# mikwieczorek/centroids-reid

Measured on AMD Instinct MI355X. Metric: train_images_per_sec, higher is better.
Workload: dtype bf16; 1 GPU; ResNet50 256x128 CTL training step: fwd+bwd, centroid-triplet + center + xent, Adam + center SGD (BASELINE configs[1]); P=16, K=4, global_batch=64, num_classes=751, parallelism=single

## Files before the change

centroids-reid_amd/csrc/elementwise.hip:

```cpp
#include "conv_common.hpp"

template <typename T> struct Vec16;
template <> struct Vec16<float> {
  static constexpr int N = 4;
  static __device__ __forceinline__ void load(const float* p, float (&v)[4]) {
    const float4 t = *reinterpret_cast<const float4*>(p); v[0] = t.x; v[1] = t.y; v[2] = t.z; v[3] = t.w;
  }
  static __device__ __forceinline__ void store(float* p, const float (&v)[4]) {
    *reinterpret_cast<float4*>(p) = make_float4(v[0], v[1], v[2], v[3]);
  }
  static __device__ __forceinline__ float rnd(float v) { return v; }
};
template <> struct Vec16<unsigned short> {
  static constexpr int N = 8;
  static __device__ __forceinline__ void load(const unsigned short* p, float (&v)[8]) {
    const uint4 t = *reinterpret_cast<const uint4*>(p);
    const unsigned w[4] = {t.x, t.y, t.z, t.w};
#pragma unroll
    for (int i = 0; i < 4; ++i) { v[2 * i] = __uint_as_float(w[i] << 16); v[2 * i + 1] = __uint_as_float(w[i] & 0xffff0000u); }
  }
  static __device__ __forceinline__ void store(unsigned short* p, const float (&v)[8]) {
    unsigned w[4];
#pragma unroll
    for (int i = 0; i < 4; ++i) w[i] = f32x2_to_bf16x2_bits(v[2 * i], v[2 * i + 1]);
    *reinterpret_cast<uint4*>(p) = make_uint4(w[0], w[1], w[2], w[3]);
  }
  static __device__ __forceinline__ float rnd(float v) { return bf16_bits_to_f32(f32_to_bf16_bits(v)); }
};

template <> struct Vec16<_Float16> {
  static constexpr int N = 8;
  static __device__ __forceinline__ void load(const _Float16* p, float (&v)[8]) {
    const uint4 t = *reinterpret_cast<const uint4*>(p);
    const unsigned w[4] = {t.x, t.y, t.z, t.w};
#pragma unroll
    for (int i = 0; i < 4; ++i) { v[2 * i] = F16T::lo(w[i]); v[2 * i + 1] = F16T::hi(w[i]); }
  }
  static __device__ __forceinline__ void store(_Float16* p, const float (&v)[8]) {
    unsigned w[4];
#pragma unroll
    for (int i = 0; i < 4; ++i) w[i] = F16T::pack2(v[2 * i], v[2 * i + 1]);
    *reinterpret_cast<uint4*>(p) = make_uint4(w[0], w[1], w[2], w[3]);
  }
  static __device__ __forceinline__ float rnd(float v) { return (float)(_Float16)v; }
};

template <int CW>
__global__ __launch_bounds__(1024) void bn2d_finalize_kernel(const float* __restrict__ partial, int rows, int C,
                                                            double count, float* __restrict__ rmean,
                                                            float* __restrict__ rvar, int training, float momentum,
                                                            float eps, const float* __restrict__ gamma,
                                                            const float* __restrict__ beta,
                                                            float* __restrict__ mean_out,
                                                            float* __restrict__ invstd_out,
                                                            float* __restrict__ scale_shift) {
  constexpr int RG = 1024 / CW;
  __shared__ double red[16][2][CW];
  const int cl = threadIdx.x % CW, rg = threadIdx.x / CW;
  const int c = blockIdx.x * CW + cl;
  if (!training) {
    if (rg == 0 && c < C) {
      const float mu = rmean[c], is = 1.0f / sqrtf(rvar[c] + eps);
      mean_out[c] = mu; invstd_out[c] = is;
      const float sc = is * (gamma ? gamma[c] : 1.f);
      scale_shift[c] = sc; scale_shift[C + c] = (beta ? beta[c] : 0.f) - mu * sc;
    }
    return;
  }
  double s1 = 0.0, s2 = 0.0;
  if (c < C)
  {
    int r = rg;
    for (; r + 3 * RG < rows; r += 4 * RG) {
      const float a0 = partial[((int64_t)r * 2) * C + c], b0 = partial[((int64_t)r * 2 + 1) * C + c];
      const float a1 = partial[((int64_t)(r + RG) * 2) * C + c], b1 = partial[((int64_t)(r + RG) * 2 + 1) * C + c];
      const float a2 = partial[((int64_t)(r + 2 * RG) * 2) * C + c], b2 = partial[((int64_t)(r + 2 * RG) * 2 + 1) * C + c];
      const float a3 = partial[((int64_t)(r + 3 * RG) * 2) * C + c], b3 = partial[((int64_t)(r + 3 * RG) * 2 + 1) * C + c];
      s1 += ((double)a0 + (double)a1) + ((double)a2 + (double)a3);
      s2 += ((double)b0 + (double)b1) + ((double)b2 + (double)b3);
    }
    for (; r < rows; r += RG) {
      s1 += (double)partial[((int64_t)r * 2) * C + c];
      s2 += (double)partial[((int64_t)r * 2 + 1) * C + c];
    }
  }
#pragma unroll
  for (int o = CW; o < 64; o <<= 1) { s1 += __shfl_xor(s1, o, 64); s2 += __shfl_xor(s2, o, 64); }
  if ((threadIdx.x & 63) < CW) { red[threadIdx.x >> 6][0][cl] = s1; red[threadIdx.x >> 6][1][cl] = s2; }
  float p_gamma = 1.f, p_beta = 0.f, p_rm = 0.f, p_rv = 0.f;
  if (rg == 0 && c < C) {
    if (gamma) p_gamma = gamma[c];
    if (beta) p_beta = beta[c];
    if (rmean) p_rm = rmean[c];
    if (rvar) p_rv = rvar[c];
  }
  __syncthreads();
  if (rg == 0 && c < C) {
    s1 = 0.0; s2 = 0.0;
#pragma unroll
    for (int q = 0; q < 16; ++q) { s1 += red[q][0][cl]; s2 += red[q][1][cl]; }
    const double mean = s1 / count;
    double var = s2 / count - mean * mean;
    if (var < 0.0) var = 0.0;
    const float mu = (float)mean, is = (float)(1.0 / sqrt(var + (double)eps));
    mean_out[c] = mu;
    invstd_out[c] = is;
    const float sc = is * p_gamma;
    scale_shift[c] = sc; scale_shift[C + c] = p_beta - mu * sc;
    if (rmean) rmean[c] = (1.f - momentum) * p_rm + momentum * (float)mean;
    if (rvar) rvar[c] = (1.f - momentum) * p_rv + momentum * (float)(count > 1.0 ? var * count / (count - 1.0) : var);
  }
}

template <typename T>
__global__ __launch_bounds__(256) void col_stats_kernel(const T* __restrict__ x, int64_t M, int C, int rows_per_block,
                                                        float* __restrict__ partial) {
  constexpr int V = Vec16<T>::N;
  __shared__ float red[2][256 * V];
  const int cpr = C / V, cw = cpr < 32 ? cpr : 32, nrl = 256 / cw;
  const int cch = threadIdx.x % cw, rl = threadIdx.x / cw;
  const int c0 = (blockIdx.x * cw + cch) * V;
  const int64_t r0 = (int64_t)blockIdx.y * rows_per_block, r1 = min(M, r0 + rows_per_block);
  float s1[V], s2[V];
#pragma unroll
  for (int k = 0; k < V; ++k) { s1[k] = 0.f; s2[k] = 0.f; }
  if (c0 < C)
    for (int64_t r = r0 + rl; r < r1; r += nrl) {
// ... 473 lines not shown
__device__ __forceinline__ void store_taps(uint8_t* p, const uint8_t (&bi)[V]) {
  static_assert(V == 4 || V == 8, "16-byte vectors of 4- or 2-byte elements");
  uint32_t lo = (uint32_t)bi[0] | ((uint32_t)bi[1] << 8) | ((uint32_t)bi[2] << 16) | ((uint32_t)bi[3] << 24);
  if constexpr (V == 4) {
    *reinterpret_cast<uint32_t*>(p) = lo;
  } else {
    uint32_t hi = (uint32_t)bi[4] | ((uint32_t)bi[5] << 8) | ((uint32_t)bi[6] << 16) | ((uint32_t)bi[7] << 24);
    *reinterpret_cast<uint2*>(p) = make_uint2(lo, hi);
  }
}
template <typename T>
__global__ __launch_bounds__(256) void maxpool_fwd_kernel(const T* __restrict__ x, int B, int H, int W, int C,
                                                          T* __restrict__ y, uint8_t* __restrict__ idx) {
  constexpr int V = Vec16<T>::N;
  const int OH = H / 2, OW = W / 2, cpr = C / V;
  const int64_t total = (int64_t)B * OH * OW * cpr;
  for (int64_t i = (int64_t)blockIdx.x * 256 + threadIdx.x; i < total; i += (int64_t)gridDim.x * 256) {
    int cc, ox, oy, b;
    if (total < (int64_t)1 << 31) {
      const unsigned u = (unsigned)i, q1 = u / (unsigned)cpr, q2 = q1 / (unsigned)OW;
      cc = (int)(u - q1 * cpr); ox = (int)(q1 - q2 * OW); b = (int)(q2 / (unsigned)OH); oy = (int)(q2 - (unsigned)b * OH);
    } else {
      cc = (int)(i % cpr);
      int64_t p = i / cpr;
      ox = (int)(p % OW); p /= OW;
      oy = (int)(p % OH);
      b = (int)(p / OH);
    }
    float best[V];
    uint8_t bi[V];
#pragma unroll
    for (int k = 0; k < V; ++k) { best[k] = -INFINITY; bi[k] = 0; }
#pragma unroll
    for (int r = 0; r < 3; ++r)
#pragma unroll
      for (int s = 0; s < 3; ++s) {
        const int iy = oy * 2 + r - 1, ix = ox * 2 + s - 1;
        if ((unsigned)iy < (unsigned)H && (unsigned)ix < (unsigned)W) {
          float v[V];
          Vec16<T>::load(x + (((int64_t)b * H + iy) * W + ix) * C + cc * V, v);
#pragma unroll
          for (int k = 0; k < V; ++k)
            if (v[k] > best[k]) { best[k] = v[k]; bi[k] = (uint8_t)(r * 3 + s); }
        }
      }
    Vec16<T>::store(y + i * V, best);
    if (idx) store_taps<V>(idx + i * V, bi);
  }
}

template <typename T>
__global__ __launch_bounds__(256) void bn_apply_maxpool_kernel(const T* __restrict__ x, const float* __restrict__ scale_shift,
                                                               int relu, int B, int H, int W, int C, T* __restrict__ y,
                                                               uint8_t* __restrict__ idx) {
  constexpr int V = Vec16<T>::N;
  const int OH = H / 2, OW = W / 2, cpr = C / V;
  const int64_t total = (int64_t)B * OH * OW * cpr;
  for (int64_t i = (int64_t)blockIdx.x * 256 + threadIdx.x; i < total; i += (int64_t)gridDim.x * 256) {
    int cc, ox, oy, b;
    if (total < (int64_t)1 << 31) {
      const unsigned u = (unsigned)i, q1 = u / (unsigned)cpr, q2 = q1 / (unsigned)OW;
      cc = (int)(u - q1 * cpr); ox = (int)(q1 - q2 * OW); b = (int)(q2 / (unsigned)OH); oy = (int)(q2 - (unsigned)b * OH);
    } else {
      cc = (int)(i % cpr);
      int64_t p = i / cpr;
      ox = (int)(p % OW); p /= OW;
      oy = (int)(p % OH);
      b = (int)(p / OH);
    }
    float sc[V], sh[V], best[V];
    uint8_t bi[V];
#pragma unroll
    for (int k = 0; k < V; ++k) { sc[k] = scale_shift[cc * V + k]; sh[k] = scale_shift[C + cc * V + k]; best[k] = -INFINITY; bi[k] = 0; }
#pragma unroll
    for (int r = 0; r < 3; ++r)
#pragma unroll
      for (int s = 0; s < 3; ++s) {
        const int iy = oy * 2 + r - 1, ix = ox * 2 + s - 1;
        if ((unsigned)iy < (unsigned)H && (unsigned)ix < (unsigned)W) {
          float v[V];
          Vec16<T>::load(x + (((int64_t)b * H + iy) * W + ix) * C + cc * V, v);
#pragma unroll
          for (int k = 0; k < V; ++k) {
            float yv = fmaf(v[k], sc[k], sh[k]);
            if (relu) yv = fmaxf(yv, 0.f);
            yv = Vec16<T>::rnd(yv);
            if (yv > best[k]) { best[k] = yv; bi[k] = (uint8_t)(r * 3 + s); }
          }
        }
      }
    Vec16<T>::store(y + i * V, best);
    if (idx) store_taps<V>(idx + i * V, bi);
  }
}

template <typename T>
__global__ __launch_bounds__(256) void maxpool_bwd_kernel(const T* __restrict__ dy, const uint8_t* __restrict__ idx,
                                                          int B, int H, int W, int C, T* __restrict__ dx) {
  constexpr int V = Vec16<T>::N;
  const int OH = H / 2, OW = W / 2, cpr = C / V;
  const int row = blockIdx.x;
  const int b = row / H, iy = row - b * H;
  T* drow = dx + (int64_t)row * W * C;
  const int nr = (iy & 1) ? 2 : 1;
  const int rr0 = (iy & 1) ? 0 : 1, rstep = 2;
  for (int par = 0; par < 2; ++par) {
    const int ns = par ? 2 : 1, ss0 = par ? 0 : 1;
    for (int v = threadIdx.x; v < (W / 2) * cpr; v += 256) {
      const int ix = 2 * (v / cpr) + par, cc = v % cpr;
      float acc[V];
#pragma unroll
      for (int k = 0; k < V; ++k) acc[k] = 0.f;
      for (int ri = 0; ri < nr; ++ri) {
        const int r = rr0 + ri * rstep, oy = (iy + 1 - r) >> 1;
        if (oy >= OH) continue;
        for (int si = 0; si < ns; ++si) {
          const int sx = ss0 + si * 2, ox = (ix + 1 - sx) >> 1;
          if (ox >= OW) continue;
          const int64_t o = ((((int64_t)b * OH + oy) * OW + ox) * cpr + cc) * V;
          float g[V];
          Vec16<T>::load(dy + o, g);
          uint8_t tap[V];
          if constexpr (V == 8) *reinterpret_cast<uint2*>(tap) = *reinterpret_cast<const uint2*>(idx + o);
          else *reinterpret_cast<unsigned*>(tap) = *reinterpret_cast<const unsigned*>(idx + o);
          const uint8_t want = (uint8_t)(r * 3 + sx);
#pragma unroll
          for (int k = 0; k < V; ++k) acc[k] += (tap[k] == want) ? g[k] : 0.f;
        }
      }
      Vec16<T>::store(drow + ((int64_t)ix * cpr + cc) * V, acc);
    }
  }
}

template <typename T>
__global__ __launch_bounds__(256) void gap_fwd_kernel(const T* __restrict__ x, int HW, int C, float* __restrict__ out,
                                                      int64_t* __restrict__ counter) {
  constexpr int V = Vec16<T>::N;
  __shared__ float red[8][32][V + 1];
  if (counter && blockIdx.x == 0 && blockIdx.y == 0 && threadIdx.x == 0) *counter += 1;
  const int cl = threadIdx.x & 31, rl = threadIdx.x >> 5;
  const int b = blockIdx.y, cc = blockIdx.x * 32 + cl;
  const bool live = cc * V < C;
  float acc[V];
#pragma unroll
  for (int k = 0; k < V; ++k) acc[k] = 0.f;
  if (live) {
    const T* p = x + (int64_t)b * HW * C + cc * V;
    for (int i = rl; i < HW; i += 8) {
      float v[V];
      Vec16<T>::load(p + (int64_t)i * C, v);
#pragma unroll
      for (int k = 0; k < V; ++k) acc[k] += v[k];
    }
  }
#pragma unroll
  for (int k = 0; k < V; ++k) red[rl][cl][k] = acc[k];
  __syncthreads();
  for (int e = threadIdx.x; e < 32 * V; e += 256) {
    const int c2 = e / V, k = e - c2 * V;
    const int ch = (blockIdx.x * 32 + c2) * V + k;
    if (ch < C) {
      float a = 0.f;
#pragma unroll
      for (int q = 0; q < 8; ++q) a += red[q][c2][k];
      out[(int64_t)b * C + ch] = a / (float)HW;
    }
  }
}

template <typename T>
__global__ __launch_bounds__(256) void gap_bwd_kernel(const float* __restrict__ dfeat, int HW, int C, int64_t total_chunks,
                                                      T* __restrict__ dx) {
  constexpr int V = Vec16<T>::N;
  const int cpr = C / V;
  const float inv = 1.0f / (float)HW;
  for (int64_t i = (int64_t)blockIdx.x * 256 + threadIdx.x; i < total_chunks; i += (int64_t)gridDim.x * 256) {
    int cc;
    int64_t b;
    if (total_chunks < (int64_t)1 << 31) { const unsigned u = (unsigned)i; cc = (int)(u % (unsigned)cpr); b = u / (unsigned)(cpr * HW); }
    else { cc = (int)(i % cpr); b = i / ((int64_t)cpr * HW); }
    float v[V];
#pragma unroll
    for (int k = 0; k < V; ++k) v[k] = dfeat[b * C + cc * V + k] * inv;
    Vec16<T>::store(dx + i * V, v);
  }
}

__device__ __forceinline__ void store_px4(float* p, const float (&v)[4]) { *reinterpret_cast<float4*>(p) = make_float4(v[0], v[1], v[2], v[3]); }
__device__ __forceinline__ void store_px4(unsigned short* p, const float (&v)[4]) {
  *reinterpret_cast<uint2*>(p) = make_uint2(Bf16T::pack2(v[0], v[1]), Bf16T::pack2(v[2], v[3]));
}
__device__ __forceinline__ void store_px4(_Float16* p, const float (&v)[4]) {
  *reinterpret_cast<uint2*>(p) = make_uint2(F16T::pack2(v[0], v[1]), F16T::pack2(v[2], v[3]));
}
template <typename T>
__global__ __launch_bounds__(256) void image_pad_kernel(const float* __restrict__ x, int B, int H, int W, T* __restrict__ y) {
  const int PH = H + 8, PW = W + 6;
  const int rows = B * PH;
  constexpr int RB = 8;
  if ((W & 3) == 0) {
    const int G = W / 4 + 2;
    for (int row0 = blockIdx.x * RB; row0 < rows; row0 += gridDim.x * RB) {
      const int n = min(RB, rows - row0) * G;
      for (int e = threadIdx.x; e < n; e += 256) {
        const int rl = e / G, gq = e - rl * G, row = row0 + rl;
        const int b = row / PH, py = row - b * PH, iy = py - 3;
        T* dst = y + (int64_t)row * PW * 4;
        const float z[4] = {0.f, 0.f, 0.f, 0.f};
        if (gq == 0 || gq == G - 1) {
          T* d = dst + (gq == 0 ? 0 : (W + 3) * 4);
          store_px4(d, z); store_px4(d + 4, z); store_px4(d + 8, z);
          continue;
// ... 184 lines not shown
  unsigned short* krsc = reinterpret_cast<unsigned short*>(e.krsc);
  unsigned short* crsk = reinterpret_cast<unsigned short*>(e.crsk);
  for (int tap = 0; tap < taps; ++tap) {
#pragma unroll
    for (int k = 0; k < 4; ++k) {
      const int o = o0 + ty + 8 * k, c = c0 + tx;
      tl[ty + 8 * k][tx] = (o < e.O && c < e.I) ? e.w[((int64_t)o * e.I + c) * taps + tap] : 0.f;
    }
    __syncthreads();
#pragma unroll
    for (int k = 0; k < 4; ++k) {
      const int o = o0 + ty + 8 * k, c = c0 + tx;
      if (o < e.O && c < e.I) {
        const int64_t d = ((int64_t)o * taps + tap) * e.I + c;
        x3_split_bits(tl[ty + 8 * k][tx], krsc + d, krsc + plane + d);
      }
      const int c2 = c0 + ty + 8 * k, o2 = o0 + tx;
      if (c2 < e.I && o2 < e.O) {
        const int64_t d = ((int64_t)c2 * taps + tap) * e.O + o2;
        x3_split_bits(tl[tx][ty + 8 * k], crsk + d, crsk + plane + d);
      }
    }
    __syncthreads();
  }
}

template <typename T>
__global__ __launch_bounds__(256) void stem_weight_prep_kernel(const float* __restrict__ w, T* __restrict__ out) {
  const int i = blockIdx.x * 256 + threadIdx.x;
  if (i >= 64 * 256) return;
  const int o = i >> 8, k = i & 255, r = k >> 5, s = (k & 31) >> 2, c = k & 3;
  const float v = (r < 7 && s < 7 && c < 3) ? w[((o * 3 + c) * 7 + r) * 7 + s] : 0.f;
  ElemIO<T>::st(out + i, v);
}

template <typename T>
__global__ __launch_bounds__(256) void nhwc_to_nchw_kernel(const T* __restrict__ x, int B, int HW, int C, float* __restrict__ y) {
  const int64_t total = (int64_t)B * HW * C;
  for (int64_t i = (int64_t)blockIdx.x * 256 + threadIdx.x; i < total; i += (int64_t)gridDim.x * 256) {
    const int p = (int)(i % HW);
    const int c = (int)((i / HW) % C);
    const int64_t b = i / ((int64_t)HW * C);
    y[i] = ElemIO<T>::ld(x + (b * HW + p) * C + c);
  }
}

static inline unsigned ew_blocks_cap(int64_t total_threads_needed, int64_t mult, int64_t cap) {
  int64_t b = (total_threads_needed + 255) / 256;
  if (b > cap) b = cap;
  if (b < 1) b = 1;
  const int64_t q = mult > 256 ? mult / 256 : 1;
  b = (b + q - 1) / q * q;
  return (unsigned)b;
}
static inline int64_t ew_env_cap() {
  static const int64_t cap = [] { const char* e = getenv("CREID_EW_BLOCKS"); const int v = e ? atoi(e) : 0; return (int64_t)(v > 0 ? v : 0); }();
  return cap;
}
static inline unsigned ew_blocks(int64_t total_threads_needed, int64_t mult) {
  const int64_t e = ew_env_cap();
  return ew_blocks_cap(total_threads_needed, mult, e > 0 ? e : 2048);
}
template <auto KERNEL>
static inline unsigned ew_blocks_k(int64_t total_threads_needed, int64_t mult) {
  static const int64_t resident = [] {
    int per_cu = 0, dev = 0, ncu = 256;
    if (hipOccupancyMaxActiveBlocksPerMultiprocessor(&per_cu, KERNEL, 256, 0) != hipSuccess || per_cu <= 0) per_cu = 8;
    (void)hipGetDevice(&dev);
    if (hipDeviceGetAttribute(&ncu, hipDeviceAttributeMultiprocessorCount, dev) != hipSuccess || ncu <= 0) ncu = 256;
    return (int64_t)per_cu * ncu;
  }();
  const int64_t e = ew_env_cap();
  return ew_blocks_cap(total_threads_needed, mult, e > 0 ? e : resident);
}

#define DISPATCH_T(dtype, EXPR_F32, EXPR_BF16, EXPR_F16) \
  do {                                                  \
    if ((dtype) == CREID_F32) { EXPR_F32; }             \
    else if ((dtype) == CREID_BF16) { EXPR_BF16; }      \
    else if ((dtype) == CREID_F16) { EXPR_F16; }        \
    else return CREID_E_DTYPE;                          \
  } while (0)

static bool fin_dry(int bit) {
  static const int v = creid_ablation_env("CREID_BN_FIN_DRY");
  return (v & bit) != 0;
}
extern "C" {

int creid_bn2d_finalize(const float* partial, int64_t rows, int64_t C, int64_t count, float* running_mean,
                        float* running_var, int training, float momentum, float eps, const float* gamma,
                        const float* beta, float* mean_out, float* invstd_out, float* scale_shift, void* stream) {
  CREID_CHECK_ARG(C > 0 && mean_out && invstd_out && scale_shift &&
                  (training ? (partial && rows > 0 && count > 0) : (running_mean && running_var)));
  if (!fin_dry(1)) {
    if (C <= 256 && rows >= 512)
      hipLaunchKernelGGL(bn2d_finalize_kernel<4>, dim3((unsigned)((C + 3) / 4)), dim3(1024), 0, as_stream(stream), partial,
                         (int)rows, (int)C, (double)count, running_mean, running_var, training, momentum, eps, gamma, beta,
                         mean_out, invstd_out, scale_shift);
    else
      hipLaunchKernelGGL(bn2d_finalize_kernel<16>, dim3((unsigned)((C + 15) / 16)), dim3(1024), 0, as_stream(stream), partial,
                         (int)rows, (int)C, (double)count, running_mean, running_var, training, momentum, eps, gamma, beta,
                         mean_out, invstd_out, scale_shift);
  }
  CREID_LAUNCH_RET();
}

int64_t creid_col_stats_rows(int64_t M) { int64_t r = (M + 127) / 128; return r < 1 ? 1 : r; }

int creid_col_stats(const void* x, int64_t M, int64_t C, int dtype, float* partial, void* stream) {
  CREID_CHECK_ARG(x && partial && M > 0 && C > 0 && C % 8 == 0);
  const int rows = (int)creid_col_stats_rows(M);
  hipStream_t s = as_stream(stream);
  DISPATCH_T(dtype,
             hipLaunchKernelGGL(col_stats_kernel<float>, dim3((unsigned)((C / 4 + 31) / 32), rows), dim3(256), 0, s,
                                (const float*)x, M, (int)C, 128, partial),
             hipLaunchKernelGGL(col_stats_kernel<unsigned short>, dim3((unsigned)((C / 8 + 31) / 32), rows), dim3(256), 0,
                                s, (const unsigned short*)x, M, (int)C, 128, partial),
             hipLaunchKernelGGL(col_stats_kernel<_Float16>, dim3((unsigned)((C / 8 + 31) / 32), rows), dim3(256), 0,
                                s, (const _Float16*)x, M, (int)C, 128, partial));
  CREID_LAUNCH_RET();
}

int creid_bn2d_apply_mask(const void* x, const float* scale_shift, const void* residual, int relu, int64_t M, int64_t C,
                          int dtype, void* y, uint8_t* mask_out, void* stream) {
  CREID_CHECK_ARG(x && scale_shift && y && M > 0 && C > 0 && C % 8 == 0);
  if (mask_out && dtype == CREID_F32) return CREID_E_DTYPE;
  hipStream_t s = as_stream(stream);
  DISPATCH_T(dtype,
             hipLaunchKernelGGL(bn2d_apply_kernel<float>, dim3(ew_blocks_k<bn2d_apply_kernel<float>>(M * C / 4, C / 4)), dim3(256), 0, s,
                                (const float*)x, scale_shift, (const float*)residual, relu, M, (int)C, (float*)y,
                                (uint8_t*)nullptr, (const float*)nullptr),
             hipLaunchKernelGGL(bn2d_apply_kernel<unsigned short>, dim3(ew_blocks_k<bn2d_apply_kernel<unsigned short>>(M * C / 8, C / 8)), dim3(256), 0, s,
                                (const unsigned short*)x, scale_shift, (const unsigned short*)residual, relu, M,
                                (int)C, (unsigned short*)y, mask_out, (const float*)nullptr),
             hipLaunchKernelGGL(bn2d_apply_kernel<_Float16>, dim3(ew_blocks_k<bn2d_apply_kernel<_Float16>>(M * C / 8, C / 8)), dim3(256), 0, s,
                                (const _Float16*)x, scale_shift, (const _Float16*)residual, relu, M,
                                (int)C, (_Float16*)y, mask_out, (const float*)nullptr));
  CREID_LAUNCH_RET();
}

int creid_bn2d_finalize_apply_mask(const float* partial, int64_t rows, int64_t C, int64_t M, float* running_mean,
                                   float* running_var, float momentum, float eps, const float* gamma, const float* beta,
                                   float* mean_out, float* invstd_out, float* scale_shift, const void* x, const void* residual,
                                   int relu, int dtype, void* y, uint8_t* mask_out, int row_blocks, void* stream) {
  CREID_CHECK_ARG(partial && rows > 0 && C > 0 && M > 0 && mean_out && invstd_out && scale_shift && x && y);
  if (mask_out && dtype == CREID_F32) return CREID_E_DTYPE;
  const int64_t strip = dtype == CREID_F32 ? 32 : 64;
  if (C % strip != 0 || rows > 1024) return CREID_E_SHAPE;
  const int strips = (int)(C / strip);
  int rb = row_blocks > 0 ? row_blocks : (512 + strips - 1) / strips;
  if (row_blocks <= 0) { if (rb > 32) rb = 32; if (rb < 4) rb = 4; }
  int64_t rpb = ((M + rb - 1) / rb + 31) / 32 * 32;
  rb = (int)((M + rpb - 1) / rpb);
  hipStream_t s = as_stream(stream);
  const dim3 grid((unsigned)strips, (unsigned)rb);
  DISPATCH_T(dtype,
             hipLaunchKernelGGL(bn2d_fin_apply_kernel<float>, grid, dim3(256), 0, s, (const float*)x, partial, (int)rows, (int)C, M,
                                (double)M, running_mean, running_var, momentum, eps, gamma, beta, mean_out, invstd_out, scale_shift,
                                (const float*)residual, relu, (float*)y, (uint8_t*)nullptr, (int)rpb),
             hipLaunchKernelGGL(bn2d_fin_apply_kernel<unsigned short>, grid, dim3(256), 0, s, (const unsigned short*)x, partial,
                                (int)rows, (int)C, M, (double)M, running_mean, running_var, momentum, eps, gamma, beta, mean_out,
                                invstd_out, scale_shift, (const unsigned short*)residual, relu, (unsigned short*)y, mask_out,
                                (int)rpb),
             hipLaunchKernelGGL(bn2d_fin_apply_kernel<_Float16>, grid, dim3(256), 0, s, (const _Float16*)x, partial, (int)rows,
                                (int)C, M, (double)M, running_mean, running_var, momentum, eps, gamma, beta, mean_out, invstd_out,
// ... 31 lines not shown
static int bn2d_bwd_impl(const void* x, const void* g, const void* act, const uint8_t* mask, PoolGrad pg, const float* mean,
                         const float* invstd, const float* gamma, int64_t M, int64_t C, int dtype, float* partial,
                         int partial_ready, float* sums, float* dgamma_accum, float* dbeta_accum, void* dx, void* gm_out,
                         void* stream, Reduce2 r2 = Reduce2{nullptr, nullptr, nullptr, nullptr}) {
  CREID_CHECK_ARG(x && (g || pg.dy) && mean && invstd && (partial || partial_ready == 2) && sums && dx && M > 0 && C > 0 && C % 8 == 0);
  if (mask && dtype == CREID_F32) return CREID_E_DTYPE;
  const int rows = (int)creid_bn2d_bwd_rows(M);
  hipStream_t s = as_stream(stream);
  if (!partial_ready)
  DISPATCH_T(dtype,
             hipLaunchKernelGGL(bn2d_bwd_reduce_kernel<float>, dim3((unsigned)((C / 4 + 31) / 32), rows), dim3(256), 0, s,
                                (const float*)x, (const float*)g, (const float*)act, mean, invstd, M, (int)C, 128, partial,
                                (const uint8_t*)nullptr, pg),
             hipLaunchKernelGGL(bn2d_bwd_reduce_kernel<unsigned short>, dim3((unsigned)((C / 8 + 31) / 32), rows), dim3(256),
                                0, s, (const unsigned short*)x, (const unsigned short*)g, (const unsigned short*)act, mean,
                                invstd, M, (int)C, 128, partial, mask, pg),
             hipLaunchKernelGGL(bn2d_bwd_reduce_kernel<_Float16>, dim3((unsigned)((C / 8 + 31) / 32), rows), dim3(256),
                                0, s, (const _Float16*)x, (const _Float16*)g, (const _Float16*)act, mean,
                                invstd, M, (int)C, 128, partial, mask, pg));
  if (partial_ready != 2 && !fin_dry(2)) {
    if (C <= 256 && rows >= 512)
      hipLaunchKernelGGL(bn2d_bwd_finalize_kernel<4>, dim3((unsigned)((C + 3) / 4)), dim3(1024), 0, s, partial, rows, (int)C,
                         (double)M, mean, invstd, gamma, sums, dgamma_accum, dbeta_accum);
    else
      hipLaunchKernelGGL(bn2d_bwd_finalize_kernel<16>, dim3((unsigned)((C + 15) / 16)), dim3(1024), 0, s, partial, rows, (int)C,
                         (double)M, mean, invstd, gamma, sums, dgamma_accum, dbeta_accum);
  }
  if (r2.x2) {
    if (act || gm_out || pg.dy || dtype == CREID_F32) return CREID_E_ARG;
    const dim3 grid2((unsigned)((C / 8 + 31) / 32), (unsigned)rows);
    if (dtype == CREID_BF16)
      hipLaunchKernelGGL(bn2d_bwd_apply_reduce2_kernel<unsigned short>, grid2, dim3(256), 0, s, (const unsigned short*)x,
                         (const unsigned short*)g, mask, sums, M, (int)C, 128, (unsigned short*)dx, (const unsigned short*)r2.x2,
                         r2.mean2, r2.invstd2, r2.partial2);
    else
      hipLaunchKernelGGL(bn2d_bwd_apply_reduce2_kernel<_Float16>, grid2, dim3(256), 0, s, (const _Float16*)x, (const _Float16*)g,
                         mask, sums, M, (int)C, 128, (_Float16*)dx, (const _Float16*)r2.x2, r2.mean2, r2.invstd2, r2.partial2);
    CREID_LAUNCH_RET();
  }
  DISPATCH_T(dtype,
             hipLaunchKernelGGL(bn2d_bwd_apply_kernel<float>, dim3(ew_blocks_k<bn2d_bwd_apply_kernel<float>>(M * C / 4, C / 4)), dim3(256), 0, s,
                                (const float*)x, (const float*)g, (const float*)act, sums, M, (int)C,
                                (float*)dx, (float*)gm_out, (const uint8_t*)nullptr, pg),
             hipLaunchKernelGGL(bn2d_bwd_apply_kernel<unsigned short>, dim3(ew_blocks_k<bn2d_bwd_apply_kernel<unsigned short>>(M * C / 8, C / 8)), dim3(256), 0, s,
                                (const unsigned short*)x, (const unsigned short*)g, (const unsigned short*)act, sums, M,
                                (int)C, (unsigned short*)dx, (unsigned short*)gm_out, mask, pg),
             hipLaunchKernelGGL(bn2d_bwd_apply_kernel<_Float16>, dim3(ew_blocks_k<bn2d_bwd_apply_kernel<_Float16>>(M * C / 8, C / 8)), dim3(256), 0, s,
                                (const _Float16*)x, (const _Float16*)g, (const _Float16*)act, sums, M,
                                (int)C, (_Float16*)dx, (_Float16*)gm_out, mask, pg));
  CREID_LAUNCH_RET();
}

int creid_bn2d_bwd_mask(const void* x, const void* g, const void* act, const uint8_t* mask, const float* mean,
                        const float* invstd, const float* gamma, int64_t M, int64_t C, int dtype, float* partial,
                        int partial_ready, float* sums, float* dgamma_accum, float* dbeta_accum, void* dx, void* gm_out,
                        void* stream) {
  CREID_CHECK_ARG(g);
  return bn2d_bwd_impl(x, g, act, mask, PoolGrad{nullptr, nullptr, 0, 0}, mean, invstd, gamma, M, C, dtype, partial, partial_ready,
                       sums, dgamma_accum, dbeta_accum, dx, gm_out, stream);
}

int creid_bn2d_bwd_mask_reduce2(const void* x, const void* g, const uint8_t* mask, const float* mean, const float* invstd,
                                const float* gamma, int64_t M, int64_t C, int dtype, float* partial, int partial_ready, float* sums,
                                float* dgamma_accum, float* dbeta_accum, void* dx, const void* x2, const float* mean2,
                                const float* invstd2, float* partial2, void* stream) {
  CREID_CHECK_ARG(g && x2 && mean2 && invstd2 && partial2);
  if (!creid_is16(dtype)) return CREID_E_DTYPE;
  return bn2d_bwd_impl(x, g, nullptr, mask, PoolGrad{nullptr, nullptr, 0, 0}, mean, invstd, gamma, M, C, dtype, partial, partial_ready,
                       sums, dgamma_accum, dbeta_accum, dx, nullptr, stream, Reduce2{x2, mean2, invstd2, partial2});
}

int creid_bn2d_bwd_pooled(const void* x, const void* dy_pooled, const uint8_t* idx, int64_t B, int64_t H, int64_t W,
                          const void* act, const float* mean, const float* invstd, const float* gamma, int64_t C, int dtype,
                          float* partial, float* sums, float* dgamma_accum, float* dbeta_accum, void* dx, void* stream) {
  CREID_CHECK_ARG(dy_pooled && idx && B > 0 && H > 0 && W > 0 && H % 2 == 0 && W % 2 == 0);
  return bn2d_bwd_impl(x, nullptr, act, nullptr, PoolGrad{dy_pooled, idx, (int)H, (int)W}, mean, invstd, gamma, B * H * W, C, dtype,
                       partial, 0, sums, dgamma_accum, dbeta_accum, dx, nullptr, stream);
}

int creid_bn2d_apply_maxpool3x3s2(const void* x, const float* scale_shift, int relu, int64_t B, int64_t H, int64_t W, int64_t C,
                                  int dtype, void* y, uint8_t* idx, void* stream) {
  CREID_CHECK_ARG(x && scale_shift && y && idx && B > 0 && H > 0 && W > 0 && C % 8 == 0 && H % 2 == 0 && W % 2 == 0);
  hipStream_t s = as_stream(stream);
  DISPATCH_T(dtype,
             hipLaunchKernelGGL(bn_apply_maxpool_kernel<float>, dim3(ew_blocks(B * H * W * C / 16, 1)), dim3(256), 0, s,
                                (const float*)x, scale_shift, relu, (int)B, (int)H, (int)W, (int)C, (float*)y, idx),
             hipLaunchKernelGGL(bn_apply_maxpool_kernel<unsigned short>, dim3(ew_blocks(B * H * W * C / 32, 1)), dim3(256), 0, s,
                                (const unsigned short*)x, scale_shift, relu, (int)B, (int)H, (int)W, (int)C, (unsigned short*)y,
                                idx),
             hipLaunchKernelGGL(bn_apply_maxpool_kernel<_Float16>, dim3(ew_blocks(B * H * W * C / 32, 1)), dim3(256), 0, s,
                                (const _Float16*)x, scale_shift, relu, (int)B, (int)H, (int)W, (int)C, (_Float16*)y,
                                idx));
  CREID_LAUNCH_RET();
}

int creid_bn2d_bwd(const void* x, const void* g, const void* act, const float* mean, const float* invstd,
                   const float* gamma, int64_t M, int64_t C, int dtype, float* partial, int partial_ready, float* sums,
                   float* dgamma_accum, float* dbeta_accum, void* dx, void* gm_out, void* stream) {
  return creid_bn2d_bwd_mask(x, g, act, nullptr, mean, invstd, gamma, M, C, dtype, partial, partial_ready, sums, dgamma_accum,
                             dbeta_accum, dx, gm_out, stream);
}

int creid_maxpool3x3s2_fwd(const void* x, int64_t B, int64_t H, int64_t W, int64_t C, int dtype, void* y, uint8_t* idx,
                           void* stream) {
  CREID_CHECK_ARG(x && y && B > 0 && H > 0 && W > 0 && C % 8 == 0 && H % 2 == 0 && W % 2 == 0);
  hipStream_t s = as_stream(stream);
  DISPATCH_T(dtype,
             hipLaunchKernelGGL(maxpool_fwd_kernel<float>, dim3(ew_blocks(B * H * W * C / 16, 1)), dim3(256), 0, s,
                                (const float*)x, (int)B, (int)H, (int)W, (int)C, (float*)y, idx),
             hipLaunchKernelGGL(maxpool_fwd_kernel<unsigned short>, dim3(ew_blocks(B * H * W * C / 32, 1)), dim3(256), 0, s,
                                (const unsigned short*)x, (int)B, (int)H, (int)W, (int)C, (unsigned short*)y, idx),
             hipLaunchKernelGGL(maxpool_fwd_kernel<_Float16>, dim3(ew_blocks(B * H * W * C / 32, 1)), dim3(256), 0, s,
                                (const _Float16*)x, (int)B, (int)H, (int)W, (int)C, (_Float16*)y, idx));
  CREID_LAUNCH_RET();
}

int creid_maxpool3x3s2_bwd(const void* dy, const uint8_t* idx, int64_t B, int64_t H, int64_t W, int64_t C, int dtype,
                           void* dx, void* stream) {
  CREID_CHECK_ARG(dy && dx && idx && B > 0 && H > 0 && W > 0 && C % 8 == 0);
  hipStream_t s = as_stream(stream);
  DISPATCH_T(dtype,
             hipLaunchKernelGGL(maxpool_bwd_kernel<float>, dim3((unsigned)(B * H)), dim3(256), 0, s,
                                (const float*)dy, idx, (int)B, (int)H, (int)W, (int)C, (float*)dx),
             hipLaunchKernelGGL(maxpool_bwd_kernel<unsigned short>, dim3((unsigned)(B * H)), dim3(256), 0, s,
                                (const unsigned short*)dy, idx, (int)B, (int)H, (int)W, (int)C, (unsigned short*)dx),
             hipLaunchKernelGGL(maxpool_bwd_kernel<_Float16>, dim3((unsigned)(B * H)), dim3(256), 0, s,
                                (const _Float16*)dy, idx, (int)B, (int)H, (int)W, (int)C, (_Float16*)dx));
  CREID_LAUNCH_RET();
}

static int gap_fwd_impl(const void* x, int64_t B, int64_t HW, int64_t C, int dtype, float* feat, int64_t* counter, void* stream) {
  CREID_CHECK_ARG(x && feat && B > 0 && HW > 0 && C % 8 == 0);
  hipStream_t s = as_stream(stream);
  DISPATCH_T(dtype,
             hipLaunchKernelGGL(gap_fwd_kernel<float>, dim3((unsigned)((C / 4 + 31) / 32), (unsigned)B), dim3(256), 0, s,
                                (const float*)x, (int)HW, (int)C, feat, counter),
             hipLaunchKernelGGL(gap_fwd_kernel<unsigned short>, dim3((unsigned)((C / 8 + 31) / 32), (unsigned)B),
                                dim3(256), 0, s, (const unsigned short*)x, (int)HW, (int)C, feat, counter),
             hipLaunchKernelGGL(gap_fwd_kernel<_Float16>, dim3((unsigned)((C / 8 + 31) / 32), (unsigned)B),
                                dim3(256), 0, s, (const _Float16*)x, (int)HW, (int)C, feat, counter));
  CREID_LAUNCH_RET();
}

int creid_gap_fwd(const void* x, int64_t B, int64_t HW, int64_t C, int dtype, float* feat, void* stream) {
  return gap_fwd_impl(x, B, HW, C, dtype, feat, nullptr, stream);
}

int creid_gap_fwd_count(const void* x, int64_t B, int64_t HW, int64_t C, int dtype, float* feat, int64_t* forward_counter,
                        void* stream) {
  CREID_CHECK_ARG(forward_counter);
  return gap_fwd_impl(x, B, HW, C, dtype, feat, forward_counter, stream);
}

int creid_gap_bwd(const float* dfeat, int64_t B, int64_t HW, int64_t C, int dtype, void* dx, void* stream) {
  CREID_CHECK_ARG(dfeat && dx && B > 0 && HW > 0 && C % 8 == 0);
  hipStream_t s = as_stream(stream);
  DISPATCH_T(dtype,
             hipLaunchKernelGGL(gap_bwd_kernel<float>, dim3(ew_blocks(B * HW * C / 4, 1)), dim3(256), 0, s, dfeat, (int)HW,
                                (int)C, B * HW * C / 4, (float*)dx),
             hipLaunchKernelGGL(gap_bwd_kernel<unsigned short>, dim3(ew_blocks(B * HW * C / 8, 1)), dim3(256), 0, s, dfeat,
                                (int)HW, (int)C, B * HW * C / 8, (unsigned short*)dx),
             hipLaunchKernelGGL(gap_bwd_kernel<_Float16>, dim3(ew_blocks(B * HW * C / 8, 1)), dim3(256), 0, s, dfeat,
                                (int)HW, (int)C, B * HW * C / 8, (_Float16*)dx));
  CREID_LAUNCH_RET();
}

int creid_image_to_nhwc4_pad(const float* x_nchw, int64_t B, int64_t H, int64_t W, int dtype, void* xpad, void* stream) {
  CREID_CHECK_ARG(x_nchw && xpad && B > 0 && H > 0 && W > 0);
  hipStream_t s = as_stream(stream);
  const int64_t total = B * (H + 8) * (W + 6);
  DISPATCH_T(dtype,
             hipLaunchKernelGGL(image_pad_kernel<float>, dim3(ew_blocks(total, 1)), dim3(256), 0, s, x_nchw, (int)B, (int)H,
                                (int)W, (float*)xpad),
             hipLaunchKernelGGL(image_pad_kernel<unsigned short>, dim3(ew_blocks(total, 1)), dim3(256), 0, s, x_nchw, (int)B,
                                (int)H, (int)W, (unsigned short*)xpad),
             hipLaunchKernelGGL(image_pad_kernel<_Float16>, dim3(ew_blocks(total, 1)), dim3(256), 0, s, x_nchw, (int)B,
                                (int)H, (int)W, (_Float16*)xpad));
  CREID_LAUNCH_RET();
}

int creid_weight_prep(const float* w_oihw, int64_t O, int64_t I, int64_t kh, int64_t kw, int dtype, void* w_krsc,
                      void* w_crsk, void* stream) {
  CREID_CHECK_ARG(w_oihw && w_krsc && O > 0 && I > 0 && kh > 0 && kw > 0);
  hipStream_t s = as_stream(stream);
  const int64_t total = O * I * kh * kw;
  if (dtype == CREID_BF16X3) {
    CREID_CHECK_ARG(!w_crsk);
    hipLaunchKernelGGL(weight_prep_x3_kernel, dim3(ew_blocks(total, 1)), dim3(256), 0, s, w_oihw, (int)O, (int)I, (int)kh,
                       (int)kw, (unsigned short*)w_krsc);
    CREID_LAUNCH_RET();
  }
  DISPATCH_T(dtype,
             hipLaunchKernelGGL(weight_prep_kernel<float>, dim3(ew_blocks(total, 1)), dim3(256), 0, s, w_oihw, (int)O, (int)I,
                                (int)kh, (int)kw, (float*)w_krsc, (float*)w_crsk),
             hipLaunchKernelGGL(weight_prep_kernel<unsigned short>, dim3(ew_blocks(total, 1)), dim3(256), 0, s, w_oihw,
                                (int)O, (int)I, (int)kh, (int)kw, (unsigned short*)w_krsc, (unsigned short*)w_crsk),
             hipLaunchKernelGGL(weight_prep_kernel<_Float16>, dim3(ew_blocks(total, 1)), dim3(256), 0, s, w_oihw,
                                (int)O, (int)I, (int)kh, (int)kw, (_Float16*)w_krsc, (_Float16*)w_crsk));
  CREID_LAUNCH_RET();
}

int64_t creid_weight_prep_entry_bytes(void) { return (int64_t)sizeof(WPrepEntry); }

int creid_weight_prep_multi(const void* table_dev, const int32_t* tile_start_dev, int64_t n_entries, int64_t total_tiles,
                            int dtype, void* stream) {
  CREID_CHECK_ARG(table_dev && tile_start_dev && n_entries > 0 && total_tiles > 0);
  hipStream_t s = as_stream(stream);
  if (dtype == CREID_BF16X3) {
    hipLaunchKernelGGL(weight_prep_multi_x3_kernel, dim3((unsigned)total_tiles), dim3(256), 0, s, (const WPrepEntry*)table_dev,
// ... 486 lines not shown
```

Measured before the change: 10790 images/s.

## Stage BN-apply rows in LDS for maxpool fwd; restructure maxpool bwd per 2x2 output

Adds a fused BN-apply+ReLU+maxpool forward kernel where each block loads 2R+1 input rows once into shared memory with an XOR swizzle, applies scale/shift there, then computes the 3x3 stride-2 max from LDS. The old kernel reloaded each input element up to nine times. The maxpool backward kernel now handles two input rows per block and gathers each dy/idx element once per 2x2 output patch, where it used to re-read them per input pixel. The forward path is on by default behind an env knob, requires a power-of-two channel-vector count, and uses up to 64KB of LDS per block, which may limit occupancy.

Measured after the change: 10810 images/s, median of 2. Within noise of the previous version (+0.2%).

```diff
diff --git a/centroids-reid_amd/csrc/elementwise.hip b/centroids-reid_amd/csrc/elementwise.hip
--- a/centroids-reid_amd/csrc/elementwise.hip
+++ b/centroids-reid_amd/csrc/elementwise.hip
@@ -10,6 +10,12 @@
     *reinterpret_cast<float4*>(p) = make_float4(v[0], v[1], v[2], v[3]);
   }
   static __device__ __forceinline__ float rnd(float v) { return v; }
+  static __device__ __forceinline__ uint4 pack(const float (&v)[4]) {
+    return make_uint4(__float_as_uint(v[0]), __float_as_uint(v[1]), __float_as_uint(v[2]), __float_as_uint(v[3]));
+  }
+  static __device__ __forceinline__ void unpack(const uint4 t, float (&v)[4]) {
+    v[0] = __uint_as_float(t.x); v[1] = __uint_as_float(t.y); v[2] = __uint_as_float(t.z); v[3] = __uint_as_float(t.w);
+  }
 };
 template <> struct Vec16<unsigned short> {
   static constexpr int N = 8;
@@ -26,6 +32,15 @@
     *reinterpret_cast<uint4*>(p) = make_uint4(w[0], w[1], w[2], w[3]);
   }
   static __device__ __forceinline__ float rnd(float v) { return bf16_bits_to_f32(f32_to_bf16_bits(v)); }
+  static __device__ __forceinline__ uint4 pack(const float (&v)[8]) {
+    return make_uint4(f32x2_to_bf16x2_bits(v[0], v[1]), f32x2_to_bf16x2_bits(v[2], v[3]), f32x2_to_bf16x2_bits(v[4], v[5]),
+                      f32x2_to_bf16x2_bits(v[6], v[7]));
+  }
+  static __device__ __forceinline__ void unpack(const uint4 t, float (&v)[8]) {
+    const unsigned w[4] = {t.x, t.y, t.z, t.w};
+#pragma unroll
+    for (int i = 0; i < 4; ++i) { v[2 * i] = __uint_as_float(w[i] << 16); v[2 * i + 1] = __uint_as_float(w[i] & 0xffff0000u); }
+  }
 };
 
 template <> struct Vec16<_Float16> {
@@ -43,6 +58,14 @@
     *reinterpret_cast<uint4*>(p) = make_uint4(w[0], w[1], w[2], w[3]);
   }
   static __device__ __forceinline__ float rnd(float v) { return (float)(_Float16)v; }
+  static __device__ __forceinline__ uint4 pack(const float (&v)[8]) {
+    return make_uint4(F16T::pack2(v[0], v[1]), F16T::pack2(v[2], v[3]), F16T::pack2(v[4], v[5]), F16T::pack2(v[6], v[7]));
+  }
+  static __device__ __forceinline__ void unpack(const uint4 t, float (&v)[8]) {
+    const unsigned w[4] = {t.x, t.y, t.z, t.w};
+#pragma unroll
+    for (int i = 0; i < 4; ++i) { v[2 * i] = F16T::lo(w[i]); v[2 * i + 1] = F16T::hi(w[i]); }
+  }
 };
 
 template <int CW>
@@ -682,7 +705,7 @@
           Vec16<T>::load(x + (((int64_t)b * H + iy) * W + ix) * C + cc * V, v);
 #pragma unroll
           for (int k = 0; k < V; ++k) {
-            float yv = fmaf(v[k], sc[k], sh[k]);
+            float yv = fmaf(v[k], sc[k], sh[k]) + 0.f;
             if (relu) yv = fmaxf(yv, 0.f);
             yv = Vec16<T>::rnd(yv);
             if (yv > best[k]) { best[k] = yv; bi[k] = (uint8_t)(r * 3 + s); }
@@ -695,40 +718,132 @@
 }
 
 template <typename T>
+__global__ __launch_bounds__(256) void bn_apply_maxpool_rows_kernel(const T* __restrict__ x, const float* __restrict__ scale_shift,
+                                                                    int relu, int H, int W, int C, int cpr_log2, int R,
+                                                                    T* __restrict__ y, uint8_t* __restrict__ idx) {
+  constexpr int V = Vec16<T>::N;
+  extern __shared__ uint4 pool_rows[];
+  const int OH = H / 2, OW = W / 2, cpr = 1 << cpr_log2, rowvecs = W << cpr_log2;
+  const int runs = (OH + R - 1) / R;
+  const int b = blockIdx.x / runs, oy0 = (blockIdx.x - b * runs) * R;
+  const int nout = min(R, OH - oy0), nin = 2 * nout + 1;
+  const int cc = threadIdx.x & (cpr - 1);
+  float sc[V], sh[V];
+#pragma unroll
+  for (int k = 0; k < V; k += 4) {
+    const float4 a = *reinterpret_cast<const float4*>(scale_shift + cc * V + k);
+    const float4 d = *reinterpret_cast<const float4*>(scale_shift + C + cc * V + k);
+    sc[k] = a.x; sc[k + 1] = a.y; sc[k + 2] = a.z; sc[k + 3] = a.w;
+    sh[k] = d.x; sh[k + 1] = d.y; sh[k + 2] = d.z; sh[k + 3] = d.w;
+  }
+  const int64_t vbase = ((int64_t)b * H + (2 * oy0 - 1)) * rowvecs;
+  const int first = oy0 == 0 ? rowvecs : 0, total = nin * rowvecs;
+  constexpr int PU = 5;
+  for (int v0 = first + threadIdx.x; v0 < total; v0 += 256 * PU) {
+    uint4 raw[PU];
+#pragma unroll
+    for (int u = 0; u < PU; ++u)
+      if (v0 + 256 * u < total) raw[u] = *reinterpret_cast<const uint4*>(x + (vbase + v0 + 256 * u) * V);
+#pragma unroll
+    for (int u = 0; u < PU; ++u) {
+      const int a = v0 + 256 * u;
+      if (a < total) {
+        float v[V];
+        Vec16<T>::unpack(raw[u], v);
+#pragma unroll
+        for (int k = 0; k < V; ++k) {
+          float yv = fmaf(v[k], sc[k], sh[k]) + 0.f;
+          if (relu) yv = fmaxf(yv, 0.f);
+          v[k] = yv;
+        }
+        pool_rows[a ^ (((a >> (cpr_log2 + 1)) & 1) << cpr_log2)] = Vec16<T>::pack(v);
+      }
+    }
+  }
+  __syncthreads();
+  for (int q = 0; q < nout; ++q) {
+    const int oy = oy0 + q;
+    for (int e = threadIdx.x; e < (OW << cpr_log2); e += 256) {
+      const int ox = e >> cpr_log2;
+      float best[V];
+      uint8_t bi[V];
+#pragma unroll
+      for (int k = 0; k < V; ++k) { best[k] = -INFINITY; bi[k] = 0; }
+#pragma unroll
+      for (int r = 0; r < 3; ++r)
+#pragma unroll
+        for (int t = 0; t < 3; ++t) {
+          const int iy = oy * 2 + r - 1, ix = ox * 2 + t - 1;
+          if ((unsigned)iy < (unsigned)H && (unsigned)ix < (unsigned)W) {
+            const int a = (2 * q + r) * rowvecs + (ix << cpr_log2) + cc;
+            float v[V];
+            Vec16<T>::unpack(pool_rows[a ^ (((a >> (cpr_log2 + 1)) & 1) << cpr_log2)], v);
+#pragma unroll
+            for (int k = 0; k < V; ++k)
+              if (v[k] > best[k]) { best[k] = v[k]; bi[k] = (uint8_t)(r * 3 + t); }
+          }
+        }
+      const int64_t i = ((int64_t)b * OH + oy) * (OW << cpr_log2) + e;
+      Vec16<T>::store(y + i * V, best);
+      if (idx) store_taps<V>(idx + i * V, bi);
+    }
+  }
+}
+
+template <typename T>
 __global__ __launch_bounds__(256) void maxpool_bwd_kernel(const T* __restrict__ dy, const uint8_t* __restrict__ idx,
                                                           int B, int H, int W, int C, T* __restrict__ dx) {
   constexpr int V = Vec16<T>::N;
-  const int OH = H / 2, OW = W / 2, cpr = C / V;
-  const int row = blockIdx.x;
-  const int b = row / H, iy = row - b * H;
-  T* drow = dx + (int64_t)row * W * C;
-  const int nr = (iy & 1) ? 2 : 1;
-  const int rr0 = (iy & 1) ? 0 : 1, rstep = 2;
-  for (int par = 0; par < 2; ++par) {
-    const int ns = par ? 2 : 1, ss0 = par ? 0 : 1;
-    for (int v = threadIdx.x; v < (W / 2) * cpr; v += 256) {
-      const int ix = 2 * (v / cpr) + par, cc = v % cpr;
-      float acc[V];
-#pragma unroll
-      for (int k = 0; k < V; ++k) acc[k] = 0.f;
-      for (int ri = 0; ri < nr; ++ri) {
-        const int r = rr0 + ri * rstep, oy = (iy + 1 - r) >> 1;
-        if (oy >= OH) continue;
-        for (int si = 0; si < ns; ++si) {
-          const int sx = ss0 + si * 2, ox = (ix + 1 - sx) >> 1;
-          if (ox >= OW) continue;
-          const int64_t o = ((((int64_t)b * OH + oy) * OW + ox) * cpr + cc) * V;
-          float g[V];
-          Vec16<T>::load(dy + o, g);
-          uint8_t tap[V];
-          if constexpr (V == 8) *reinterpret_cast<uint2*>(tap) = *reinterpret_cast<const uint2*>(idx + o);
-          else *reinterpret_cast<unsigned*>(tap) = *reinterpret_cast<const unsigned*>(idx + o);
-          const uint8_t want = (uint8_t)(r * 3 + sx);
-#pragma unroll
-          for (int k = 0; k < V; ++k) acc[k] += (tap[k] == want) ? g[k] : 0.f;
+  const int OH = H / 2, OW = W / 2, cpr = C / V, HP = (H + 1) / 2;
+  const int b = blockIdx.x / HP, m = blockIdx.x - b * HP;
+  const int iy0 = 2 * m;
+  const bool row1 = iy0 + 1 < H;
+  T* drow = dx + ((int64_t)b * H + iy0) * W * C;
+  for (int v = threadIdx.x; v < (W / 2) * cpr; v += 256) {
+    const int px = v / cpr, cc = v - px * cpr;
+    uint4 graw[2][2];
+    uint2 traw[2][2];
+    bool ok[2][2];
+#pragma unroll
+    for (int i = 0; i < 2; ++i)
+#pragma unroll
+      for (int j = 0; j < 2; ++j) {
+        ok[i][j] = m + i < OH && px + j < OW && (i == 0 || row1);
+        if (ok[i][j]) {
+          const int64_t o = ((((int64_t)b * OH + m + i) * OW + px + j) * cpr + cc) * V;
+          graw[i][j] = *reinterpret_cast<const uint4*>(dy + o);
+          if constexpr (V == 8) traw[i][j] = *reinterpret_cast<const uint2*>(idx + o);
+          else traw[i][j] = make_uint2(*reinterpret_cast<const unsigned*>(idx + o), 0u);
         }
       }
-      Vec16<T>::store(drow + ((int64_t)ix * cpr + cc) * V, acc);
+    float g[2][2][V];
+#pragma unroll
+    for (int i = 0; i < 2; ++i)
+#pragma unroll
+      for (int j = 0; j < 2; ++j)
+        if (ok[i][j]) Vec16<T>::unpack(graw[i][j], g[i][j]);
+    auto add = [&](float (&acc)[V], int i, int j, unsigned want) {
+      if (ok[i][j]) {
+#pragma unroll
+        for (int k = 0; k < V; ++k) {
+          const unsigned tap = ((k < 4 ? traw[i][j].x : traw[i][j].y) >> (8 * (k & 3))) & 0xffu;
+          acc[k] += (tap == want) ? g[i][j][k] : 0.f;
+        }
+      }
+    };
+    float a00[V], a01[V], a10[V], a11[V];
+#pragma unroll
+    for (int k = 0; k < V; ++k) { a00[k] = 0.f; a01[k] = 0.f; a10[k] = 0.f; a11[k] = 0.f; }
+    add(a00, 0, 0, 4u);
+    add(a01, 0, 1, 3u); add(a01, 0, 0, 5u);
+    add(a10, 1, 0, 1u); add(a10, 0, 0, 7u);
+    add(a11, 1, 1, 0u); add(a11, 1, 0, 2u); add(a11, 0, 1, 6u); add(a11, 0, 0, 8u);
+    T* d0 = drow + ((int64_t)(2 * px) * cpr + cc) * V;
+    Vec16<T>::store(d0, a00);
+    Vec16<T>::store(d0 + (int64_t)cpr * V, a01);
+    if (row1) {
+      Vec16<T>::store(d0 + (int64_t)W * C, a10);
+      Vec16<T>::store(d0 + (int64_t)W * C + (int64_t)cpr * V, a11);
     }
   }
 }
@@ -1079,6 +1194,10 @@
     else return CREID_E_DTYPE;                          \
   } while (0)
 
+static bool pool_rows_on() {
+  const char* e = CREID_KNOB_ENV("CREID_POOL_ROWS");
+  return !(e && e[0] == '0');
+}
 static bool fin_dry(int bit) {
   static const int v = creid_ablation_env("CREID_BN_FIN_DRY");
   return (v & bit) != 0;
@@ -1276,6 +1395,27 @@
                                   int dtype, void* y, uint8_t* idx, void* stream) {
   CREID_CHECK_ARG(x && scale_shift && y && idx && B > 0 && H > 0 && W > 0 && C % 8 == 0 && H % 2 == 0 && W % 2 == 0);
   hipStream_t s = as_stream(stream);
+  {
+    const int64_t V = dtype == CREID_F32 ? 4 : 8, cpr = C / V, rowbytes = W * cpr * 16;
+    int lg = 0;
+    while (((int64_t)1 << lg) < cpr) ++lg;
+    int R = 2;
+    if (5 * rowbytes > 65536) R = 1;
+    const int64_t runs = (H / 2 + R - 1) / R;
+    if (pool_rows_on() && C % V == 0 && ((int64_t)1 << lg) == cpr && cpr <= 256 && (2 * R + 1) * rowbytes <= 65536 &&
+        B * runs < ((int64_t)1 << 31)) {
+      const unsigned lds = (unsigned)((2 * R + 1) * rowbytes);
+      const dim3 grid((unsigned)(B * runs));
+      DISPATCH_T(dtype,
+                 hipLaunchKernelGGL(bn_apply_maxpool_rows_kernel<float>, grid, dim3(256), lds, s, (const float*)x, scale_shift, relu,
+                                    (int)H, (int)W, (int)C, lg, R, (float*)y, idx),
+                 hipLaunchKernelGGL(bn_apply_maxpool_rows_kernel<unsigned short>, grid, dim3(256), lds, s, (const unsigned short*)x,
+                                    scale_shift, relu, (int)H, (int)W, (int)C, lg, R, (unsigned short*)y, idx),
+                 hipLaunchKernelGGL(bn_apply_maxpool_rows_kernel<_Float16>, grid, dim3(256), lds, s, (const _Float16*)x, scale_shift,
+                                    relu, (int)H, (int)W, (int)C, lg, R, (_Float16*)y, idx));
+      CREID_LAUNCH_RET();
+    }
+  }
   DISPATCH_T(dtype,
              hipLaunchKernelGGL(bn_apply_maxpool_kernel<float>, dim3(ew_blocks(B * H * W * C / 16, 1)), dim3(256), 0, s,
                                 (const float*)x, scale_shift, relu, (int)B, (int)H, (int)W, (int)C, (float*)y, idx),
@@ -1314,11 +1454,11 @@
   CREID_CHECK_ARG(dy && dx && idx && B > 0 && H > 0 && W > 0 && C % 8 == 0);
   hipStream_t s = as_stream(stream);
   DISPATCH_T(dtype,
-             hipLaunchKernelGGL(maxpool_bwd_kernel<float>, dim3((unsigned)(B * H)), dim3(256), 0, s,
+             hipLaunchKernelGGL(maxpool_bwd_kernel<float>, dim3((unsigned)(B * ((H + 1) / 2))), dim3(256), 0, s,
                                 (const float*)dy, idx, (int)B, (int)H, (int)W, (int)C, (float*)dx),
-             hipLaunchKernelGGL(maxpool_bwd_kernel<unsigned short>, dim3((unsigned)(B * H)), dim3(256), 0, s,
+             hipLaunchKernelGGL(maxpool_bwd_kernel<unsigned short>, dim3((unsigned)(B * ((H + 1) / 2))), dim3(256), 0, s,
                                 (const unsigned short*)dy, idx, (int)B, (int)H, (int)W, (int)C, (unsigned short*)dx),
-             hipLaunchKernelGGL(maxpool_bwd_kernel<_Float16>, dim3((unsigned)(B * H)), dim3(256), 0, s,
+             hipLaunchKernelGGL(maxpool_bwd_kernel<_Float16>, dim3((unsigned)(B * ((H + 1) / 2))), dim3(256), 0, s,
                                 (const _Float16*)dy, idx, (int)B, (int)H, (int)W, (int)C, (_Float16*)dx));
   CREID_LAUNCH_RET();
 }
```
